# aik2mlj/polyffusion

Hardware: AMD Instinct MI355X
Metric: denoising steps/sec (8-bar prmat2c, batch 16) (higher is better)
Workload: dtype bf16x3; 1 GPU; sdf_chd8bar cond generation, batch 16 per GPU, 1000-step DDPM sampler loop body (BASELINE.json configs[1]); weights: deterministic synthetic, 41.08M params; global_batch=16, parallelism=batch-shard x1

## Files before the change

polyffusion_amd/csrc/conv_bf16x3.hip:

```cpp
#include <vector>

#include "conv_common.h"

namespace pf {

#ifdef PF_TRACE
__device__ unsigned long long g_trace[8192];
#define TR() do { if (trace_on && tslot < 2040) { g_trace[tbase + tslot++] = __builtin_amdgcn_s_memtime(); } } while (0)
#else
#define TR() do {} while (0)
#endif

typedef x3_t x3x4 __attribute__((ext_vector_type(4)));

template <int KS, int STRIDE, int TWIN, int BN>
constexpr int conv_bf3_row_pitch() {
  return (KS != 1 && STRIDE == 1 && BN >= 128) ? (TWIN * 40 + 127) / 128 * 128 : TWIN * 40;
}

#ifndef PF_KG2_RING
#define PF_KG2_RING 5
#endif
template <int KS, int BN, int KG>
constexpr bool conv_bf3_pingpong() { return KS == 3 && BN == 128 && KG == 2; }
template <int KS, int KG, int BN = 64>
constexpr int conv_bf3_wring() { return KS == 3 ? (KG == 2 && !conv_bf3_pingpong<KS, BN, KG>() ? PF_KG2_RING : 3) : 2; }

template <int KS, int STRIDE, int TH, int TW, int BN, bool SKIP, int KG = 1>
constexpr size_t conv_bf3_group_lds() {
  constexpr int THIN = (TH - 1) * STRIDE + KS, TWIN = (TW - 1) * STRIDE + KS;
  constexpr int NABUF = (KS == 1) ? 2 : 1, WRING = conv_bf3_wring<KS, KG, BN>();
  constexpr size_t main_b = (size_t)(2 * NABUF * THIN * conv_bf3_row_pitch<KS, STRIDE, TWIN, BN>() + WRING * 8 * BN * 8) * 2;
  constexpr int NB1 = BN >= 128 ? 2 : 1;
  constexpr size_t skip_b = SKIP ? (size_t)(2 * NB1 * TH * TW * 40 + NB1 * 8 * BN * 8) * 2 : 0;
  return main_b > skip_b ? main_b : skip_b;
}

template <int KS, int STRIDE, bool UPS, int TH, int TW, int BN, int PRO, int NWM, bool SKIP, int KG = 1>
__global__ __launch_bounds__(KG * NWM * 128, 2) void conv_bf3_kernel(ConvP p) {
  constexpr int NT = NWM * 128;
  constexpr int BK = 32;
  constexpr int BM = TH * TW;
  constexpr int THIN = (TH - 1) * STRIDE + KS;
  constexpr int TWIN = (TW - 1) * STRIDE + KS;
  constexpr int NPIX = THIN * TWIN;
  constexpr int PITCH = BK + 8;
  constexpr int KQ = BK / 4;
  constexpr int TOTA = NPIX * KQ;
  constexpr int NA = (TOTA + NT - 1) / NT;
  constexpr int PSTEP = NT / KQ;
  constexpr int TOTW = 8 * BN;
  constexpr int NW = TOTW / NT;
  constexpr int TAPS = KS * KS;
  constexpr int NABUF = (KS == 1) ? 2 : 1;
  constexpr int WRING = conv_bf3_wring<KS, KG, BN>();
  constexpr int WM = BM / NWM, WN = BN / 2;
  constexpr int FM = WM / 32, FN = WN / 32;
  constexpr int PAD = (KS == 3) ? 1 : 0;
  constexpr int RP = conv_bf3_row_pitch<KS, STRIDE, TWIN, BN>();
  constexpr int ABUF = THIN * RP;
  constexpr int APLANE = NABUF * ABUF;
  static_assert(TOTW % NT == 0 && FM >= 1 && FN >= 1, "bad tile");

  extern __shared__ __attribute__((aligned(16))) unsigned char smem_all[];
  const int kg = KG == 1 ? 0 : __builtin_amdgcn_readfirstlane(threadIdx.x / NT);
  unsigned char* smem_raw = smem_all + kg * conv_bf3_group_lds<KS, STRIDE, TH, TW, BN, SKIP, KG>();
  x3_t* sAh = reinterpret_cast<x3_t*>(smem_raw);
  x3_t* sAl = sAh + APLANE;
  x3_t* sW = sAl + APLANE;

  const int tid = KG == 1 ? threadIdx.x : threadIdx.x % NT, lane = tid & 63;
  const int wave = __builtin_amdgcn_readfirstlane(tid >> 6);
#ifdef PF_TRACE
  const bool trace_on = (threadIdx.x == 0) && (blockIdx.x == 0 || blockIdx.x == 301 || blockIdx.x == gridDim.x - 1);
  const int tbase = blockIdx.x == 0 ? 0 : (blockIdx.x == 301 ? 2048 : 4096);
  int tslot = 0;
  TR();
#endif
  const int wm = wave >> 1, wn = wave & 1;

  const int nwg = gridDim.x;
  int lid;
  {
    const int orig = blockIdx.x;
    const int xcd = orig & 7, q = nwg >> 3, r = nwg & 7;
    lid = (xcd < r ? xcd * (q + 1) : r * (q + 1) + (xcd - r) * q) + (orig >> 3);
  }
  int q = 0;
  if constexpr (KS == 2) { q = lid & 3; lid >>= 2; p.fold_py = q >> 1; p.fold_px = q & 1; }
  int t = fdiv(lid, p.d_ks);
  const int sidx = lid - t * p.ksplit;
  lid = t;
  int mt = fdiv(lid, p.d_nt);
  const int nti = lid - mt * p.nt;
  t = fdiv(mt, p.d_tx);
  const int tx = mt - t * p.tiles_x; mt = t;
  const int b = fdiv(mt, p.d_ty);
  const int ty = mt - b * p.tiles_y;
  const int n0 = nti * BN;
  const int oy0 = ty * TH, ox0 = tx * TW;
  conv_shared_x1(p, b);
  const int ppad = p.x1_bmod > 0 ? (b - b % p.x1_bmod) * p.Hin * p.Win : 0;
  const int iy0 = KS == 2 ? oy0 - 1 + (q >> 1) : oy0 * STRIDE - PAD, ix0 = KS == 2 ? ox0 - 1 + (q & 1) : ox0 * STRIDE - PAD;
  const int Hlog = UPS ? 2 * p.Hin : p.Hin, Wlog = UPS ? 2 * p.Win : p.Win;
  const int cin = p.c0 + p.c1;
  const int K8 = cin / 8;
  const int nsl = p.ksplit * KG, sl = sidx * KG + kg;
  const bool pow2 = (nsl & (nsl - 1)) == 0;
  const int nsh = 31 - __builtin_clz(nsl);
  const int cbeg = pow2 ? ((cin / BK) * sl) >> nsh : (cin / BK) * sl / nsl;
  const int nchunk = (pow2 ? ((cin / BK) * (sl + 1)) >> nsh : (cin / BK) * (sl + 1) / nsl) - cbeg;

  const int c4 = tid % KQ;
  int poff[NA];
  float pmu[NA], prs[NA];
#pragma unroll
  for (int i = 0; i < NA; ++i) {
    const int pix = tid / KQ + i * PSTEP;
    poff[i] = -1; pmu[i] = 0.f; prs[i] = 0.f;
    if (pix < NPIX) {
      const int hy = pix / TWIN, hx = pix % TWIN;
      const int iy = iy0 + hy, ix = ix0 + hx;
      if (iy >= 0 && iy < Hlog && ix >= 0 && ix < Wlog) {
        const int sy = UPS ? (iy >> 1) : iy, sx = UPS ? (ix >> 1) : ix;
        poff[i] = (b * p.Hin + sy) * p.Win + sx;
        if (PRO == 3) { pmu[i] = p.mean[poff[i]]; prs[i] = p.rstd[poff[i]]; }
      }
    }
  }

  f32x4 ra[NA], vsc, vsh;
  u32x4 rw[NW];
  vsc = f32x4{1.f, 1.f, 1.f, 1.f}; vsh = f32x4{0.f, 0.f, 0.f, 0.f};

  bool sc_ready = !((PRO == 1 || PRO == 2) && p.gn_s0);
  auto loadA = [&](int chunk) {
    const int cg = (cbeg + chunk) * BK;
    const float* src; int cs, co;
    if (cg < p.c0) { src = p.x0; cs = p.c0; co = cg; } else { src = p.x1; cs = p.c1; co = cg - p.c0; }
#pragma unroll
    for (int i = 0; i < NA; ++i) {
      if (KS != 1 || poff[i] >= 0) ra[i] = *reinterpret_cast<const f32x4*>(src + co + (unsigned)(max(poff[i], ppad) * cs + c4 * 4));
      else ra[i] = f32x4{0.f, 0.f, 0.f, 0.f};
    }
    if (PRO == 1 || PRO == 2) {
      const float* scp = sc_ready ? p.sc + (size_t)b * cin : p.gn_gamma;
      const float* shp = sc_ready ? p.sh + (size_t)b * cin : p.gn_beta;
      vsc = *reinterpret_cast<const f32x4*>(scp + cg + c4 * 4);
      vsh = *reinterpret_cast<const f32x4*>(shp + cg + c4 * 4);
    } else if (PRO == 3) {
      vsc = *reinterpret_cast<const f32x4*>(p.sc + cg + c4 * 4);
      vsh = *reinterpret_cast<const f32x4*>(p.sh + cg + c4 * 4);
    }
  };
  x3x4 qh[NA], ql[NA];
  auto transformPiece = [&](int i) {
    {
      f32x4 v = ra[i];
      if (poff[i] < 0) v = f32x4{0.f, 0.f, 0.f, 0.f};
      else if (PRO != 0) {
        if (PRO == 3) {
          v = (v - pmu[i]) * prs[i] * vsc + vsh;
        } else {
          v = v * vsc + vsh;
          if (PRO == 1) { v[0] = silu_f(v[0]); v[1] = silu_f(v[1]); v[2] = silu_f(v[2]); v[3] = silu_f(v[3]); }
        }
      }
      qh[i] = __builtin_convertvector(v, x3x4);
      const f32x4 hf = __builtin_convertvector(qh[i], f32x4);
      ql[i] = __builtin_convertvector(v - hf, x3x4);
    }
  };
  auto transformA = [&]() {
#pragma unroll
    for (int i = 0; i < NA; ++i) transformPiece(i);
  };
  auto writeA = [&](int buf) {
#pragma unroll
    for (int i = 0; i < NA; ++i) {
      const int pix = tid / KQ + i * PSTEP;
      if (pix < NPIX) {
        const int o = buf * ABUF + (pix / TWIN) * RP + (pix % TWIN) * PITCH + c4 * 4;
        *reinterpret_cast<x3x4*>(sAh + o) = qh[i];
        *reinterpret_cast<x3x4*>(sAl + o) = ql[i];
      }
    }
  };
  auto storeA = [&](int buf) { transformA(); writeA(buf); };
  auto loadW = [&](int chunk, int tap) {
    const size_t toff = ((size_t)tap * K8 + (size_t)(cbeg + chunk) * 4) * ((size_t)2 * p.Npad * 8);
#pragma unroll
    for (int j = 0; j < NW; ++j) {
      const int u = tid + j * NT;
      const int k8l = u / (2 * BN), plane = (u / BN) & 1, n = u % BN;
      rw[j] = *reinterpret_cast<const u32x4*>(static_cast<const x3_t*>(p.w) + ((size_t)(k8l * 2 + plane) * p.Npad + n0 + n) * 8 + toff);
    }
  };
  auto storeW = [&](int buf) {
    x3_t* dst = sW + buf * (TOTW * 8);
#pragma unroll
    for (int j = 0; j < NW; ++j) {
      *reinterpret_cast<u32x4*>(dst + (tid + j * NT) * 8) = rw[j];
    }
  };

  static_assert(NT % (2 * BN) == 0, "pieces of a thread must be whole k8 rows apart");
  const int wrow_b = 2 * p.Npad * 8 * 2;
  const __amdgpu_buffer_rsrc_t rsW = dma_resource(static_cast<const x3_t*>(p.w) + (size_t)n0 * 8);
  const int vw0 = (((tid / (2 * BN)) * 2 + ((tid / BN) & 1)) * p.Npad + tid % BN) * 16;
  auto gldsW = [&](int chunk, int tap, int buf) {
    const int toff = ((q * TAPS + tap) * K8 + (cbeg + chunk) * 4) * wrow_b;
#pragma unroll
    for (int j = 0; j < NW; ++j) {
      x3_t* l = sW + buf * (TOTW * 8) + (wave * 64 + j * NT) * 8;
      dma16(rsW, vw0, toff + j * (NT / (2 * BN)) * wrow_b, l);
    }
  };

  int hbase[FM];
#pragma unroll
  for (int fm = 0; fm < FM; ++fm) {
    const int pp = wm * WM + fm * 32 + (lane & 31);
    const int py = pp / TW, px = pp % TW;
    hbase[fm] = (py * STRIDE) * RP + (px * STRIDE) * PITCH + 8 * (lane >> 5);
  }
  const int wbase = ((lane >> 5) * 2 * BN + wn * WN + (lane & 31)) * 8;

  f32x16 acc[FM][FN];
#pragma unroll
  for (int fm = 0; fm < FM; ++fm)
#pragma unroll
    for (int fn = 0; fn < FN; ++fn)
#pragma unroll
      for (int r = 0; r < 16; ++r) acc[fm][fn][r] = 0.f;


  auto gnFused = [&]() {
    if constexpr (PRO == 1 || PRO == 2) {
      if (p.gn_s0) {
        gn_fused_prologue<KG * NT>(p, b, threadIdx.x, p.Hin * p.Win, reinterpret_cast<double*>(smem_all));
        const int cg = cbeg * BK;
        vsc = *reinterpret_cast<const f32x4*>(p.sc + (size_t)b * cin + cg + c4 * 4);
        vsh = *reinterpret_cast<const f32x4*>(p.sh + (size_t)b * cin + cg + c4 * 4);
        sc_ready = true;
      }
    }
  };
  if constexpr (KS == 1) {
    loadA(0); loadW(0, 0);
    gnFused();
    storeA(0); storeW(0);
    __syncthreads();
    for (int chunk = 0; chunk < nchunk; ++chunk) {
      const int nchunk1 = min(chunk + 1, nchunk - 1);
      loadW(nchunk1, 0);
      loadA(nchunk1);
      const int aoff = (chunk & 1) * ABUF;
      const x3_t* cW = sW + (chunk & 1) * (TOTW * 8) + wbase;
#pragma unroll
      for (int s = 0; s < BK / 16; ++s) {
        x3x8 ah[FM], al[FM], bh[FN], bl[FN];
#pragma unroll
        for (int fm = 0; fm < FM; ++fm) {
          ah[fm] = *reinterpret_cast<const x3x8*>(sAh + aoff + hbase[fm] + s * 16);
          al[fm] = *reinterpret_cast<const x3x8*>(sAl + aoff + hbase[fm] + s * 16);
        }
#pragma unroll
        for (int fn = 0; fn < FN; ++fn) {
          bh[fn] = *reinterpret_cast<const x3x8*>(cW + ((4 * s) * BN + fn * 32) * 8);
          bl[fn] = *reinterpret_cast<const x3x8*>(cW + ((4 * s + 1) * BN + fn * 32) * 8);
        }
#pragma unroll
        for (int fm = 0; fm < FM; ++fm)
#pragma unroll
          for (int fn = 0; fn < FN; ++fn) acc[fm][fn] = x3_mfma_32x32x16(al[fm], bh[fn], acc[fm][fn], 0, 0, 0);
#pragma unroll
        for (int fm = 0; fm < FM; ++fm)
#pragma unroll
          for (int fn = 0; fn < FN; ++fn) acc[fm][fn] = x3_mfma_32x32x16(ah[fm], bl[fn], acc[fm][fn], 0, 0, 0);
#pragma unroll
        for (int fm = 0; fm < FM; ++fm)
#pragma unroll
          for (int fn = 0; fn < FN; ++fn) acc[fm][fn] = x3_mfma_32x32x16(ah[fm], bh[fn], acc[fm][fn], 0, 0, 0);
      }
      storeW((chunk + 1) & 1);
      storeA((chunk + 1) & 1);
      __syncthreads();
    }
  } else {
    constexpr int NS = BK / 16;
    static_assert(NS == 2 && WRING >= 2 && WRING <= TAPS, "pipeline is written for two K steps per tap and a ring no deeper than a chunk's taps");
    constexpr bool DYN = TAPS % WRING != 0;
    constexpr int NAL = NA + (PRO != 0 ? 2 : 0);
    constexpr bool PP = conv_bf3_pingpong<KS, BN, KG>();
#pragma unroll
    for (int d = 0; d < (PP ? 2 : WRING); ++d) gldsW(0, d, d);
    TR();
    loadA(0);
    TR();
    gnFused();
    storeA(0);
    TR();
    asm volatile("s_waitcnt vmcnt(0) lgkmcnt(0)" ::: "memory");
    __builtin_amdgcn_s_barrier();
    x3x8 ah[FM], al[FM], bh[FN], bl[FN];
    unsigned abase[FM];
#pragma unroll
    for (int fm = 0; fm < FM; ++fm) abase[fm] = (unsigned)(size_t)(__attribute__((address_space(3))) x3_t*)(sAh + hbase[fm]);
    const unsigned wb = (unsigned)(size_t)(__attribute__((address_space(3))) x3_t*)(sW + wbase);
    constexpr int ALO = APLANE * 2;
    constexpr int WSLOT = TOTW * 16;
    static_assert(ALO + (2 * RP + 2 * PITCH) * 2 + 64 < 65536 && (DYN ? 1 : WRING) * WSLOT < 65536, "LDS immediates must fit 16 bits");
#define LD_AL1(I, AOFF, S) al[I] = lds_read128<ALO + ((AOFF) + (S) * 16) * 2>(abase[I])
#define LD_AH1(I, AOFF, S) ah[I] = lds_read128<((AOFF) + (S) * 16) * 2>(abase[I])
#define LD_BH1(I, SLOT, S) bh[I] = lds_read128<(DYN ? 0 : slot_##SLOT * WSLOT) + ((4 * (S)) * BN + (I) * 32) * 16>(DYN ? wb_##SLOT : wb)
#define LD_BL1(I, SLOT, S) bl[I] = lds_read128<(DYN ? 0 : slot_##SLOT * WSLOT) + ((4 * (S) + 1) * BN + (I) * 32) * 16>(DYN ? wb_##SLOT : wb)
#define LD_AL(AOFF, S) static_for<0, FM>([&](auto i) { LD_AL1(i.value, AOFF, S); })
#define LD_AH(AOFF, S) static_for<0, FM>([&](auto i) { LD_AH1(i.value, AOFF, S); })
#define LD_BH(SLOT, S) static_for<0, FN>([&](auto i) { LD_BH1(i.value, SLOT, S); })
#define LD_BL(SLOT, S) static_for<0, FN>([&](auto i) { LD_BL1(i.value, SLOT, S); })
#define SB() __builtin_amdgcn_sched_barrier(0)
#define FENCE() asm volatile("" ::: "memory")
    constexpr int G = FM * FN;
    auto GX = [&](auto&& f) {
      static_for<0, FM>([&](auto fm) { static_for<0, FN>([&](auto fn) {
        acc[fm.value][fn.value] = x3_mfma_32x32x16(al[fm.value], bh[fn.value], acc[fm.value][fn.value], 0, 0, 0);
        SB(); f(fm, fn); SB(); }); });
    };
    auto GZ = [&](auto&& f) {
      static_for<0, FN>([&](auto fn) { static_for<0, FM>([&](auto fm) {
        acc[fm.value][fn.value] = x3_mfma_32x32x16(ah[fm.value], bh[fn.value], acc[fm.value][fn.value], 0, 0, 0);
        SB(); f(fm, fn); SB(); }); });
    };
    auto GY = [&](auto&& f) {
      static_for<0, FM>([&](auto fm) { static_for<0, FN>([&](auto fn) {
        acc[fm.value][fn.value] = x3_mfma_32x32x16(ah[fm.value], bl[fn.value], acc[fm.value][fn.value], 0, 0, 0);
        SB(); f(fm, fn); SB(); }); });
    };
    auto loadApiece = [&](int chunk, int i) {
      const int cg = (cbeg + chunk) * BK;
      const float* src; int cs, co;
      if (cg < p.c0) { src = p.x0; cs = p.c0; co = cg; } else { src = p.x1; cs = p.c1; co = cg - p.c0; }
      if (i < NA) asm volatile("global_load_dwordx4 %0, %1, off" : "=v"(ra[i]) : "v"(src + co + (unsigned)(max(poff[i], ppad) * cs + c4 * 4)));
      else if (PRO == 1 || PRO == 2) {
        asm volatile("global_load_dwordx4 %0, %1, off" : "=v"(vsc) : "v"(p.sc + (size_t)b * cin + cg + c4 * 4));
        asm volatile("global_load_dwordx4 %0, %1, off" : "=v"(vsh) : "v"(p.sh + (size_t)b * cin + cg + c4 * 4));
      }
    };
    auto transformSub = [&](int i, int sub) {
      if (sub < 2) {
#pragma unroll
        for (int e = 2 * sub; e < 2 * sub + 2; ++e) {
          float v = ra[i][e];
          if (poff[i] < 0) v = 0.f;
          else if (PRO != 0) { v = v * vsc[e] + vsh[e]; if (PRO == 1) v = silu_f(v); }
          ra[i][e] = v;
        }
      } else if (sub == 2) {
        qh[i] = __builtin_convertvector(ra[i], x3x4);
      } else {
        ql[i] = __builtin_convertvector(ra[i] - __builtin_convertvector(qh[i], f32x4), x3x4);
      }
    };
    auto gldsWpiece = [&](int chunk, int tap, int buf, int j) {
      const int toff = ((q * TAPS + tap) * K8 + (cbeg + chunk) * 4) * wrow_b;
      x3_t* l = sW + buf * (TOTW * 8) + (wave * 64 + j * NT) * 8;
      dma16(rsW, vw0, toff + j * (NT / (2 * BN)) * wrow_b, l);
    };
    if constexpr (PP) {
      static_assert(WRING == 3 && TAPS == 9 && NS == 2, "ping-pong loop: ring of 3 over 9 taps");
      x3x8 ah2[NS][FM], al2[NS][FM], bh2[NS][FN], bl2[NS][FN];
      int woff[NA];
#pragma unroll
      for (int i = 0; i < NA; ++i) {
        const int pix = min(tid / KQ + i * PSTEP, NPIX - 1);
        woff[i] = (pix / TWIN) * RP + (pix % TWIN) * PITCH + c4 * 4;
      }
      if (kg) __builtin_amdgcn_s_barrier();
      for (int chunk = 0; chunk < nchunk; ++chunk) {
        const bool has_next = chunk + 1 < nchunk;
        const int chunkn = min(chunk + 1, nchunk - 1);
        static_for<0, TAPS>([&](auto tapc) {
          constexpr int tap = decltype(tapc)::value;
          constexpr int aoff = (tap / KS) * RP + (tap % KS) * PITCH;
          constexpr int slot_cur = tap % WRING, slot_ref = (tap + 2) % WRING;
          constexpr int T0 = 2, TSPAN = TAPS - 1 - T0;
          int c2 = chunk + (tap + 2) / TAPS, t2 = (tap + 2) % TAPS;
          if (c2 >= nchunk) { c2 = nchunk - 1; t2 = TAPS - 1; }
          TR();
          SB();
          static_for<0, NS>([&](auto sc_) {
            constexpr int st = decltype(sc_)::value;
            static_for<0, FM>([&](auto i) { al2[st][i.value] = lds_read128<ALO + (aoff + st * 16) * 2>(abase[i.value]); });
            static_for<0, FN>([&](auto i) { bh2[st][i.value] = lds_read128<slot_cur * WSLOT + ((4 * st) * BN + i.value * 32) * 16>(wb); });
            static_for<0, FM>([&](auto i) { ah2[st][i.value] = lds_read128<(aoff + st * 16) * 2>(abase[i.value]); });
            static_for<0, FN>([&](auto i) { bl2[st][i.value] = lds_read128<slot_cur * WSLOT + ((4 * st + 1) * BN + i.value * 32) * 16>(wb); });
          });
          static_for<0, NW>([&](auto jc) { gldsWpiece(c2, t2, slot_ref, decltype(jc)::value); });
          if constexpr (tap == 0) {
            static_for<0, NA + 1>([&](auto ic) { if (ic.value < NA || PRO != 0) loadApiece(chunkn, ic.value); });
          }
          if constexpr (tap == T0) {
            asm volatile("s_waitcnt vmcnt(%0)" ::"n"(2 * NW) : "memory");
            SB();
          }
          if (has_next) {
            static_for<0, NA>([&](auto ic) {
              constexpr int i = decltype(ic)::value;
              if constexpr (tap == T0 + (i * TSPAN) / NA) { static_for<0, 4>([&](auto sc_) { transformSub(i, decltype(sc_)::value); }); }
            });
          }
          SB();
          TR();
          asm volatile("s_waitcnt lgkmcnt(0)" ::: "memory");
          TR();
          __builtin_amdgcn_s_barrier();
          FENCE();
          SB();
          TR();
          static_for<0, NS>([&](auto sc_) {
            constexpr int st = decltype(sc_)::value;
            static_for<0, FM>([&](auto fm) { static_for<0, FN>([&](auto fn) {
              acc[fm.value][fn.value] = x3_mfma_32x32x16(al2[st][fm.value], bh2[st][fn.value], acc[fm.value][fn.value], 0, 0, 0);
              SB(); }); });
            static_for<0, FN>([&](auto fn) { static_for<0, FM>([&](auto fm) {
              acc[fm.value][fn.value] = x3_mfma_32x32x16(ah2[st][fm.value], bh2[st][fn.value], acc[fm.value][fn.value], 0, 0, 0);
              SB(); }); });
            static_for<0, FM>([&](auto fm) { static_for<0, FN>([&](auto fn) {
              acc[fm.value][fn.value] = x3_mfma_32x32x16(ah2[st][fm.value], bl2[st][fn.value], acc[fm.value][fn.value], 0, 0, 0);
              SB(); }); });
          });
          if constexpr (tap == TAPS - 1) {
            if (has_next) {
#pragma unroll
              for (int i = 0; i < NA; ++i) {
                if (tid / KQ + i * PSTEP < NPIX) {
                  *reinterpret_cast<x3x4*>(sAh + woff[i]) = qh[i];
                  *reinterpret_cast<x3x4*>(sAl + woff[i]) = ql[i];
                }
              }
            }
          }
          SB();
          TR();
          asm volatile("s_waitcnt vmcnt(%0) lgkmcnt(0)" ::"n"(NW + (tap < T0 ? NAL : 0)) : "memory");
          TR();
          __builtin_amdgcn_s_barrier();
          FENCE();
          SB();
        });
      }
      if (!kg) __builtin_amdgcn_s_barrier();
    } else {
    int rs_cur = 0;
    {
      constexpr int slot_cur = 0;
      const unsigned wb_cur = wb;
      (void)slot_cur; (void)wb_cur;
      LD_AL(0, 0); LD_BH(cur, 0); LD_AH(0, 0); LD_BL(cur, 0);
    }
    for (int chunk = 0; chunk < nchunk; ++chunk) {
      const bool has_next = chunk + 1 < nchunk;
      const int chunkn = min(chunk + 1, nchunk - 1);
      static_for<0, TAPS>([&](auto tapc) {
        constexpr int tap = decltype(tapc)::value;
        constexpr int aoff = (tap / KS) * RP + (tap % KS) * PITCH;
        constexpr int aoff1 = ((tap + 1) / KS) * RP + ((tap + 1) % KS) * PITCH;
        constexpr int slot_cur = DYN ? 0 : tap % WRING, slot_nxt = DYN ? 0 : (tap + 1) % WRING;
        const int rs_nxt = rs_cur + 1 == WRING ? 0 : rs_cur + 1;
        const int slot = DYN ? rs_cur : slot_cur;
        const unsigned wb_cur = wb + (unsigned)rs_cur * WSLOT, wb_nxt = wb + (unsigned)rs_nxt * WSLOT;
        (void)wb_cur; (void)wb_nxt; (void)slot_nxt;
        constexpr int T0 = TAPS >= 9 ? 2 : 1, TSPAN = TAPS - 1 - T0;
        int c2 = chunk + (tap + WRING) / TAPS, t2 = (tap + WRING) % TAPS;
        if (c2 >= nchunk) { c2 = nchunk - 1; t2 = TAPS - 1; }
        auto filler = [&](auto kc) {
          constexpr int k = decltype(kc)::value;
          if constexpr (tap == 0 && k < 3 * G) {
            static_for<0, NA + 1>([&](auto ic) {
              constexpr int i = decltype(ic)::value;
              if constexpr (k == (i * 3 * G) / (NA + 1)) { if (i < NA || PRO != 0) loadApiece(chunkn, i); }
            });
          }
          if constexpr (k >= 3 * G && k < 4 * G) {
            if constexpr (tap == T0 && k == 3 * G) {
              asm volatile("s_waitcnt vmcnt(%0)" ::"n"(T0 * NW) : "memory");
              SB();
            }
            if (has_next) {
              static_for<0, NA>([&](auto ic) {
                constexpr int i = decltype(ic)::value;
                if constexpr (tap == T0 + (i * TSPAN) / NA) {
                  static_for<0, 4>([&](auto sc_) {
                    constexpr int sub = decltype(sc_)::value;
                    if constexpr (k - 3 * G == (sub * G) / 4) transformSub(i, sub);
                  });
                }
              });
            }
          }
          if constexpr (k >= 4 * G && k < 5 * G) {
            static_for<0, NW>([&](auto jc) {
              constexpr int j = decltype(jc)::value;
              if constexpr (k - 4 * G == (j * G) / NW) gldsWpiece(c2, t2, slot, j);
            });
          }
        };
        TR();
        SB();
        lgkm_wait<(tap == 0) ? FM : FM + FN>(); SB();
        GX([&](auto fm, auto fn) {
          if constexpr (fn.value == FN - 1) LD_AL1(fm.value, aoff, 1);
          filler(std::integral_constant<int, 0 * G + fm.value * FN + fn.value>{});
        });
        lgkm_wait<(tap == 0) ? FM : FM + FN>(); SB();
        GZ([&](auto fm, auto fn) {
          if constexpr (fm.value == FM - 1) LD_BH1(fn.value, cur, 1);
          filler(std::integral_constant<int, 1 * G + fn.value * FM + fm.value>{});
        });
        lgkm_wait<FM + FN>(); SB();
        GY([&](auto fm, auto fn) {
          if constexpr (fn.value == FN - 1) LD_AH1(fm.value, aoff, 1);
          if constexpr (fm.value == FM - 1 && fn.value == FN - 1) LD_BL(cur, 1);
          filler(std::integral_constant<int, 2 * G + fm.value * FN + fn.value>{});
        });
        lgkm_wait<FM + FN>(); SB();
        GX([&](auto fm, auto fn) { filler(std::integral_constant<int, 3 * G + fm.value * FN + fn.value>{}); });
        SB();
        TR();
        asm volatile("s_waitcnt vmcnt(%0) lgkmcnt(0)" ::"n"((WRING - 2) * NW + (tap < WRING - 1 ? NAL : 0)) : "memory");
        TR();
        __builtin_amdgcn_s_barrier();
        FENCE();
        SB();
        TR();
        if constexpr (tap == TAPS - 1) {
          if (has_next) writeA(0);
          SB();
          GZ([&](auto fm, auto fn) {
            if constexpr (fm.value == FM - 1) LD_BH1(fn.value, nxt, 0);
            filler(std::integral_constant<int, 4 * G + fn.value * FM + fm.value>{});
          });
          GY([&](auto fm, auto fn) {
            if constexpr (fm.value == FM - 1 && fn.value == FN - 1) LD_BL(nxt, 0);
            filler(std::integral_constant<int, 5 * G + fm.value * FN + fn.value>{});
          });
          asm volatile("s_waitcnt lgkmcnt(0)" ::: "memory");
          __builtin_amdgcn_s_barrier();
          FENCE();
          LD_AL(0, 0); LD_AH(0, 0); SB();
        } else {
          GZ([&](auto fm, auto fn) {
            if constexpr (fn.value == 0) LD_AL1(fm.value, aoff1, 0);
            if constexpr (fm.value == FM - 1) LD_BH1(fn.value, nxt, 0);
            filler(std::integral_constant<int, 4 * G + fn.value * FM + fm.value>{});
          });
          GY([&](auto fm, auto fn) {
            if constexpr (fn.value == FN - 1) LD_AH1(fm.value, aoff1, 0);
            if constexpr (fm.value == FM - 1 && fn.value == FN - 1) LD_BL(nxt, 0);
            filler(std::integral_constant<int, 5 * G + fm.value * FN + fn.value>{});
          });
        }
        rs_cur = rs_nxt;
      });
    }
    }
#undef LD_AL1
#undef LD_AH1
#undef LD_BH1
#undef LD_BL1
#undef LD_AL
#undef LD_AH
#undef LD_BH
#undef LD_BL
#undef FENCE
#undef SB
    asm volatile("s_waitcnt vmcnt(0) lgkmcnt(0)" ::: "memory");
#pragma unroll
    for (int i = 0; i < NA; ++i) asm volatile("" : "+v"(ra[i]));
    asm volatile("" : "+v"(vsc), "+v"(vsh));
    if constexpr (!PP) {
    #pragma unroll
    for (int i = 0; i < FM; ++i) asm volatile("" ::"v"(al[i]), "v"(ah[i]));
    #pragma unroll
    for (int i = 0; i < FN; ++i) asm volatile("" ::"v"(bh[i]), "v"(bl[i]));
    }
    __builtin_amdgcn_sched_barrier(0);
  }

  if constexpr (SKIP) {
    if (sidx == 0) {
      constexpr int NB1 = BN >= 128 ? 2 : 1;
      constexpr int NA1 = BM * KQ / NT;
      static_assert(BM * KQ % NT == 0, "tile pixels must divide over the block");
      x3_t* a1h = reinterpret_cast<x3_t*>(smem_raw);
      x3_t* a1l = a1h + NB1 * BM * PITCH;
      x3_t* w1 = a1l + NB1 * BM * PITCH;
      int goff[NA1];
#pragma unroll
      for (int i = 0; i < NA1; ++i) {
        const int pix = tid / KQ + i * PSTEP;
        const int oy = oy0 + pix / TW, ox = ox0 + pix % TW;
        goff[i] = (oy < p.Hout && ox < p.Wout) ? (b * p.Hout + oy) * p.Wout + ox : -1;
      }
      f32x4 r1[NA1];
      u32x4 rw1[NW];
      auto load1 = [&](int chunk) {
        const int cg = chunk * BK;
        const float* src; int cs, co;
        if (cg < p.sc0) { src = p.sx0; cs = p.sc0; co = cg; } else { src = p.sx1; cs = p.sc1; co = cg - p.sc0; }
#pragma unroll
        for (int i = 0; i < NA1; ++i) {
          if (goff[i] >= 0) r1[i] = *reinterpret_cast<const f32x4*>(src + co + (unsigned)(goff[i] * cs + c4 * 4));
          else r1[i] = f32x4{0.f, 0.f, 0.f, 0.f};
        }
#pragma unroll
        for (int j = 0; j < NW; ++j) {
          const int u = tid + j * NT;
          const int k8l = u / (2 * BN), plane = (u / BN) & 1, n = u % BN;
          rw1[j] = *reinterpret_cast<const u32x4*>(static_cast<const x3_t*>(p.sw) + ((size_t)((chunk * 4 + k8l) * 2 + plane) * p.Npad + n0 + n) * 8);
        }
      };
      auto store1 = [&](int buf) {
#pragma unroll
        for (int i = 0; i < NA1; ++i) {
          const x3x4 hi = __builtin_convertvector(r1[i], x3x4);
          const x3x4 lo = __builtin_convertvector(r1[i] - __builtin_convertvector(hi, f32x4), x3x4);
          const int o = (buf * BM + tid / KQ + i * PSTEP) * PITCH + c4 * 4;
          *reinterpret_cast<x3x4*>(a1h + o) = hi;
          *reinterpret_cast<x3x4*>(a1l + o) = lo;
        }
#pragma unroll
        for (int j = 0; j < NW; ++j) *reinterpret_cast<u32x4*>(w1 + buf * (TOTW * 8) + (tid + j * NT) * 8) = rw1[j];
      };
      int arow[FM];
#pragma unroll
      for (int fm = 0; fm < FM; ++fm) arow[fm] = (wm * WM + fm * 32 + (lane & 31)) * PITCH + 8 * (lane >> 5);
      const int nchx = (p.sc0 + p.sc1) / BK;
      const int ch0 = nchx * kg / KG, nch1 = nchx * (kg + 1) / KG;
      load1(ch0);
      __syncthreads();
      store1(0);
      __syncthreads();
      for (int chunk = ch0; chunk < nch1; ++chunk) {
        if (chunk + 1 < nch1) load1(chunk + 1);
        const int cur = NB1 == 2 ? ((chunk - ch0) & 1) : 0;
        const int ao = cur * BM * PITCH;
        const x3_t* cW = w1 + cur * (TOTW * 8) + wbase;
#pragma unroll
        for (int s2 = 0; s2 < BK / 16; ++s2) {
          x3x8 ah[FM], al[FM], bh[FN], bl[FN];
#pragma unroll
          for (int fm = 0; fm < FM; ++fm) {
            ah[fm] = *reinterpret_cast<const x3x8*>(a1h + ao + arow[fm] + s2 * 16);
            al[fm] = *reinterpret_cast<const x3x8*>(a1l + ao + arow[fm] + s2 * 16);
          }
#pragma unroll
          for (int fn = 0; fn < FN; ++fn) {
            bh[fn] = *reinterpret_cast<const x3x8*>(cW + ((4 * s2) * BN + fn * 32) * 8);
            bl[fn] = *reinterpret_cast<const x3x8*>(cW + ((4 * s2 + 1) * BN + fn * 32) * 8);
          }
#pragma unroll
          for (int fm = 0; fm < FM; ++fm)
#pragma unroll
            for (int fn = 0; fn < FN; ++fn) acc[fm][fn] = x3_mfma_32x32x16(al[fm], bh[fn], acc[fm][fn], 0, 0, 0);
#pragma unroll
          for (int fm = 0; fm < FM; ++fm)
#pragma unroll
            for (int fn = 0; fn < FN; ++fn) acc[fm][fn] = x3_mfma_32x32x16(ah[fm], bl[fn], acc[fm][fn], 0, 0, 0);
#pragma unroll
          for (int fm = 0; fm < FM; ++fm)
#pragma unroll
            for (int fn = 0; fn < FN; ++fn) acc[fm][fn] = x3_mfma_32x32x16(ah[fm], bh[fn], acc[fm][fn], 0, 0, 0);
        }
        if constexpr (NB1 == 1) __syncthreads();
        if (chunk + 1 < nch1) store1(NB1 == 2 ? ((chunk + 1 - ch0) & 1) : 0);
        __syncthreads();
      }
    }
  }

  TR();
  if (p.partial) p.partial += (size_t)sidx * ((size_t)p.B * p.Hout * p.Wout) * p.N;
  if constexpr (KG == 2) {
    float* xch = reinterpret_cast<float*>(smem_all);
    __syncthreads();
    if (kg == 1) {
#pragma unroll
      for (int fm = 0; fm < FM; ++fm)
#pragma unroll
        for (int fn = 0; fn < FN; ++fn)
#pragma unroll
          for (int r = 0; r < 16; ++r) xch[((fm * FN + fn) * 16 + r) * NT + tid] = acc[fm][fn][r];
    }
    __syncthreads();
    if (kg == 0) {
#pragma unroll
      for (int fm = 0; fm < FM; ++fm)
#pragma unroll
        for (int fn = 0; fn < FN; ++fn)
#pragma unroll
          for (int r = 0; r < 16; ++r) acc[fm][fn][r] += xch[((fm * FN + fn) * 16 + r) * NT + tid];
    }
    __syncthreads();
  }
  x3_unscale(acc);
  conv_epilogue<TH, TW, BN, FM, FN, NWM>(p, acc, b, oy0, ox0, n0, wm, wn, lane, tid, reinterpret_cast<float*>(smem_all), kg == 0);
  TR();
}

__global__ __launch_bounds__(1024) void splitk_reduce_kernel(const float* __restrict__ part, int S, int M, int N, int hw,
                                                            const float* __restrict__ bias, const float* __restrict__ bias2,
                                                            const float* __restrict__ sbias, int ld_sb,
                                                            const long long* __restrict__ sb_rows, int sb_nrows,
                                                            const float* __restrict__ res, int ld_res, float* __restrict__ out,
                                                            int ld_out, float* __restrict__ stats, unsigned* amax) {
  __shared__ float red[16][64][2];
  const int tid = threadIdx.x, c = tid & 63, rg = tid >> 6;
  const int row0 = blockIdx.x * 64;
  const int b = row0 / hw, tile = (row0 % hw) / 64, ntiles = hw / 64;
  {
    const int n = blockIdx.y * 64 + c;
    float s1 = 0.f, s2 = 0.f;
    unsigned am = 0;
    if (n < N) {
      long long sr = b;
      if (sb_rows) { sr = sb_rows[b]; sr = sr < 0 ? 0 : (sr >= sb_nrows ? sb_nrows - 1 : sr); }
      const float cb = (bias ? bias[n] : 0.f) + (bias2 ? bias2[n] : 0.f) + (sbias ? sbias[(size_t)sr * ld_sb + n] : 0.f);
      for (int i = 0; i < 4; ++i) {
        const size_t m = row0 + rg + 16 * i;
        float v = cb;
        for (int s = 0; s < S; ++s) v += part[((size_t)s * M + m) * N + n];
        if (res) v += res[m * ld_res + n];
        out[m * ld_out + n] = v;
        amax_acc(am, v);
        s1 += v; s2 += v * v;
      }
    }
    amax_flush(amax, am);
    if (stats) {
      red[rg][c][0] = s1; red[rg][c][1] = s2;
      __syncthreads();
      if (rg == 0 && n < N) {
        float* dst = stats + (((size_t)b * ntiles + tile) * N + n) * 2;
        float a0 = 0.f, a1 = 0.f;
#pragma unroll
        for (int j = 0; j < 16; ++j) { a0 += red[j][c][0]; a1 += red[j][c][1]; }
        dst[0] = a0; dst[1] = a1;
      }
      __syncthreads();
    }
  }
}

template <int KS, int STRIDE, bool UPS, int TH, int TW, int BN, int PRO, int NWM = 2, bool SKIP = false, int KG = 1>
static int launch3_cfg(ConvP& p, hipStream_t stream) {
  constexpr int FMFN = (TH * TW / NWM / 32) * (BN / 2 / 32);
  constexpr size_t lds_groups = KG * conv_bf3_group_lds<KS, STRIDE, TH, TW, BN, SKIP, KG>();
  constexpr size_t lds_xch = KG == 2 ? (size_t)FMFN * 16 * NWM * 128 * 4 : 0;
  constexpr size_t lds = lds_groups > lds_xch ? lds_groups : lds_xch;
  static_assert(lds <= 160 * 1024, "LDS budget");
  p.tiles_x = cdiv(p.Wout, TW);
  p.tiles_y = cdiv(p.Hout, TH);
  p.nt = cdiv(p.Npad, BN);
  conv_fill_divs(p);
  auto kern = conv_bf3_kernel<KS, STRIDE, UPS, TH, TW, BN, PRO, NWM, SKIP, KG>;
  static std::atomic<uint64_t> attr_done{0};
  if (int rc = set_max_lds_once(reinterpret_cast<const void*>(kern), (int)lds, attr_done)) return rc;
  const int grid = p.B * p.tiles_y * p.tiles_x * p.nt * p.ksplit * (KS == 2 ? 4 : 1);
  hipLaunchKernelGGL(kern, dim3(grid), dim3(KG * NWM * 128), lds, stream, p);
  PF_CHECK_HIP(hipGetLastError());
  return PF_OK;
}

template <int KS, int STRIDE, bool UPS, int PRO>
static int dispatch_tile3(ConvP& p, int tile, hipStream_t s) {
  if constexpr (KS == 1) {
    if (tile == 0) return launch3_cfg<1, 1, false, 1, 128, 128, PRO>(p, s);
    if (tile == 1) return launch3_cfg<1, 1, false, 1, 128, 64, PRO>(p, s);
    return launch3_cfg<1, 1, false, 1, 64, 64, PRO>(p, s);
  } else if constexpr (KS == 2) {
    if (tile == 0) return launch3_cfg<2, 1, false, 8, 16, 128, PRO>(p, s);
    if (tile == 1) return launch3_cfg<2, 1, false, 8, 16, 64, PRO>(p, s);
    return launch3_cfg<2, 1, false, 4, 16, 64, PRO>(p, s);
  } else if constexpr (STRIDE == 2) {
    return launch3_cfg<3, 2, false, 4, 16, 64, PRO>(p, s);
  } else {
    if constexpr (!UPS && PRO == 1) {
      const int blocks = p.B * cdiv(p.Hout, tile == 3 ? 16 : tile == 2 ? 4 : 8) * cdiv(p.Wout, 16) * cdiv(p.Npad, tile == 0 ? 128 : 64);
      const int cus = num_cus();
      const bool kg2 = tile == 2 && p.ksplit == 1 && blocks <= cus && ((p.c0 + p.c1) / 32) % 2 == 0 && (!p.sw || ((p.sc0 + p.sc1) / 32) % 2 == 0);
      if (kg2) return p.sw ? launch3_cfg<3, 1, false, 4, 16, 64, 1, 2, true, 2>(p, s) : launch3_cfg<3, 1, false, 4, 16, 64, 1, 2, false, 2>(p, s);
      if (p.pp && tile == 0 && p.ksplit == 1 && blocks <= cus && (p.c0 + p.c1) >= 256 && ((p.c0 + p.c1) / 32) % 2 == 0 && (!p.sw || ((p.sc0 + p.sc1) / 32) % 2 == 0))
        return p.sw ? launch3_cfg<3, 1, false, 8, 16, 128, 1, 2, true, 2>(p, s) : launch3_cfg<3, 1, false, 8, 16, 128, 1, 2, false, 2>(p, s);
      if (tile == 3) return p.sw ? launch3_cfg<3, 1, false, 16, 16, 64, 1, 2, true>(p, s) : launch3_cfg<3, 1, false, 16, 16, 64, 1, 2, false>(p, s);
      if (p.sw) {
        if (tile == 0) return launch3_cfg<3, 1, false, 8, 16, 128, 1, 2, true>(p, s);
        if (tile == 1) return launch3_cfg<3, 1, false, 8, 16, 64, 1, 2, true>(p, s);
        return launch3_cfg<3, 1, false, 4, 16, 64, 1, 2, true>(p, s);
      }
    }
    if (tile == 0) return launch3_cfg<3, 1, UPS, 8, 16, 128, PRO>(p, s);
    if (tile == 1) return launch3_cfg<3, 1, UPS, 8, 16, 64, PRO>(p, s);
    return launch3_cfg<3, 1, UPS, 4, 16, 64, PRO>(p, s);
  }
}

int launch_conv_bf3(const pf_conv_args& a, hipStream_t stream) {
  if (conv_wino_eligible(a)) return launch_conv_wino(a, stream);
  ConvP p;
  memset(&p, 0, sizeof p);
  p.x0 = a.x0; p.x1 = a.x1; p.c0 = a.c0; p.c1 = a.c1;
  p.B = a.batch; p.Hin = a.hin; p.Win = a.win;
  p.Hout = a.hin; p.Wout = a.win;
  if (a.ups) { p.Hout *= 2; p.Wout *= 2; }
  if (a.stride == 2) { p.Hout = (p.Hout - 1) / 2 + 1; p.Wout = (p.Wout - 1) / 2 + 1; }
  p.w = a.w; p.N = a.n; p.Npad = (a.n + 63) / 64 * 64;
  p.sc = a.sc; p.sh = a.sh; p.mean = a.mean; p.rstd = a.rstd;
  p.bias = a.bias; p.sbias = a.sbias; p.ld_sbias = a.ld_sbias; p.res = a.res; p.ld_res = a.ld_res;
  p.sb_rows = reinterpret_cast<const long long*>(a.sbias_rows); p.sb_nrows = a.sbias_nrows;
  p.geglu = a.geglu; p.out = a.out; p.ld_out = a.ld_out; p.stats = a.stats_out;
  p.ksplit = conv_ksplit(a);
  p.pp = !a.no_pp;
  p.partial = p.ksplit > 1 ? static_cast<float*>(a.splitk_ws) : nullptr;
  p.qkv = a.qkv_planes; p.out_planes = a.out_planes;
  if (a.gn_stats0 && (a.prologue == 1 || a.prologue == 2)) {
    p.gn_s0 = a.gn_stats0; p.gn_t0 = a.gn_tiles0; p.gn_s1 = a.gn_stats1; p.gn_t1 = a.gn_tiles1;
    p.gn_gamma = a.gn_gamma; p.gn_beta = a.gn_beta; p.gn_eps = a.gn_eps; p.gn_groups = a.gn_groups;
  }
  p.sx0 = a.skip_x0; p.sc0 = a.skip_c0; p.sx1 = a.skip_x1; p.sc1 = a.skip_c1; p.sw = a.skip_w; p.bias2 = a.skip_w ? a.skip_bias : nullptr;
  p.x1_bmod = a.x1_bmod;
  p.amax = static_cast<unsigned*>(a.absmax_slot);
  const int tile = conv_pick_tile(a);
  if (a.ks == 1) {
    switch (a.prologue) {
      case 0: return dispatch_tile3<1, 1, false, 0>(p, tile, stream);
      case 2: return dispatch_tile3<1, 1, false, 2>(p, tile, stream);
      default: return dispatch_tile3<1, 1, false, 3>(p, tile, stream);
    }
  }
  if (a.ups_fold) {
    p.Hout = a.hin; p.Wout = a.win; p.fold = 1;
    return dispatch_tile3<2, 1, false, 0>(p, tile, stream);
  }
  if (a.stride == 2) return dispatch_tile3<3, 2, false, 0>(p, tile, stream);
  int rc = a.ups ? dispatch_tile3<3, 1, true, 0>(p, tile, stream) : dispatch_tile3<3, 1, false, 1>(p, tile, stream);
  if (rc != PF_OK || p.ksplit == 1) return rc;
  const int M = p.B * p.Hout * p.Wout;
  hipLaunchKernelGGL(splitk_reduce_kernel, dim3(M / 64, cdiv(p.N, 64)), dim3(1024), 0, stream, static_cast<const float*>(a.splitk_ws), p.ksplit, M, p.N,
                     p.Hout * p.Wout, p.bias, p.bias2, p.sbias, p.ld_sbias, p.sb_rows, p.sb_nrows, p.res, p.ld_res, p.out, p.ld_out, p.stats, p.amax);
  PF_CHECK_HIP(hipGetLastError());
  return PF_OK;
}

#ifdef PF_TRACE
extern "C" int pf_debug_trace_read(unsigned long long* dst, int n) {
  return hipMemcpyFromSymbol(dst, HIP_SYMBOL(g_trace), (size_t)n * 8) == hipSuccess ? 0 : -1;
}
extern "C" int pf_debug_trace_clear() {
  static unsigned long long z[8192];
  return hipMemcpyToSymbol(HIP_SYMBOL(g_trace), z, sizeof z) == hipSuccess ? 0 : -1;
}
#endif

static inline unsigned short f2bf_rne(float f) {
  unsigned int u; memcpy(&u, &f, 4);
  u += 0x7FFFu + ((u >> 16) & 1u);
  return (unsigned short)(u >> 16);
}
static inline float bf2f(unsigned short h) { unsigned int u = (unsigned int)h << 16; float f; memcpy(&f, &u, 4); return f; }

bool pack_gemm_bf3(void* dst_, const float* src, int n_src, int K, int taps, int Npad, int n_off, const int* colmap) {
  unsigned short* dst = (unsigned short*)dst_;
  bool fits = true;
  const int K8 = K / 8;
  for (int n = 0; n < n_src; ++n) {
    const int col = colmap ? colmap[n] : n_off + n;
    for (int k = 0; k < K; ++k)
      for (int t = 0; t < taps; ++t) {
        const float v = src[((size_t)n * K + k) * taps + t];
#ifdef PF_X3_F16
        const float vs = fminf(fmaxf(v * PF_X3_WS, -65504.f), 65504.f);
        fits = fits && vs == v * PF_X3_WS;
        const _Float16 fh = (_Float16)vs, fl = (_Float16)(vs - (float)fh);
        unsigned short hi, lo;
        memcpy(&hi, &fh, 2); memcpy(&lo, &fl, 2);
#else
        const unsigned short hi = f2bf_rne(v);
        const unsigned short lo = f2bf_rne(v - bf2f(hi));
#endif
        const size_t base = ((size_t)t * K8 + k / 8) * 2;
        dst[((base + 0) * Npad + col) * 8 + (k & 7)] = hi;
        dst[((base + 1) * Npad + col) * 8 + (k & 7)] = lo;
      }
  }
  return fits;
}


bool pack_upfold_bf3(void* dst, const float* src, int N, int K, int Npad) {
  std::vector<float> f((size_t)N * K * 16);
  static const int lo[2][2] = {{0, 1}, {0, 2}}, hi[2][2] = {{0, 2}, {1, 2}};
  for (size_t nk = 0; nk < (size_t)N * K; ++nk) {
    const float* w = src + nk * 9;
    for (int py = 0; py < 2; ++py)
      for (int px = 0; px < 2; ++px)
        for (int dy = 0; dy < 2; ++dy)
          for (int dx = 0; dx < 2; ++dx) {
            double acc = 0.0;
            for (int ky = lo[py][dy]; ky <= hi[py][dy]; ++ky)
              for (int kx = lo[px][dx]; kx <= hi[px][dx]; ++kx) acc += w[ky * 3 + kx];
            f[nk * 16 + (py * 2 + px) * 4 + dy * 2 + dx] = (float)acc;
          }
  }
  return pack_gemm_bf3(dst, f.data(), N, K, 16, Npad, 0, nullptr);
}

}
```

Baseline: 210.5 steps/s.

## Add 4-way in-block K-split with interleaved hi/lo LDS layout for conv

Adds a KG=4 variant of the 3x3 conv kernel that splits the reduction over channels across four wave groups inside one block, with hi and lo bf16 planes interleaved per row in LDS and a three-way LDS reduction of partial accumulators. It also enables the KG=2 split for stride-2 3x3 convs when the grid is smaller than the CU count. The aim is to raise per-CU parallelism on small-grid layers, at the cost of larger blocks, more LDS and an extra cross-group reduction. The interleaved layout changes bank access patterns, which may add LDS conflicts.

```diff
diff --git a/polyffusion_amd/csrc/conv_bf16x3.hip b/polyffusion_amd/csrc/conv_bf16x3.hip
--- a/polyffusion_amd/csrc/conv_bf16x3.hip
+++ b/polyffusion_amd/csrc/conv_bf16x3.hip
@@ -13,24 +13,35 @@
 
 typedef x3_t x3x4 __attribute__((ext_vector_type(4)));
 
-template <int KS, int STRIDE, int TWIN, int BN>
+template <int KG>
+constexpr bool conv_bf3_ilv() { return KG == 4; }
+template <int KS, int STRIDE, int TWIN, int BN, int KG = 1>
 constexpr int conv_bf3_row_pitch() {
+  if (conv_bf3_ilv<KG>()) return TWIN * 72;
   return (KS != 1 && STRIDE == 1 && BN >= 128) ? (TWIN * 40 + 127) / 128 * 128 : TWIN * 40;
 }
 
 #ifndef PF_KG2_RING
 #define PF_KG2_RING 5
 #endif
+#ifndef PF_KG4_RING
+#define PF_KG4_RING 3
+#endif
 template <int KS, int BN, int KG>
 constexpr bool conv_bf3_pingpong() { return KS == 3 && BN == 128 && KG == 2; }
-template <int KS, int KG, int BN = 64>
-constexpr int conv_bf3_wring() { return KS == 3 ? (KG == 2 && !conv_bf3_pingpong<KS, BN, KG>() ? PF_KG2_RING : 3) : 2; }
+template <int KS, int KG, int BN = 64, int STRIDE = 1>
+constexpr int conv_bf3_wring() {
+  if (KS != 3) return 2;
+  if (KG == 4) return PF_KG4_RING;
+  return KG == 2 && STRIDE == 1 && !conv_bf3_pingpong<KS, BN, KG>() ? PF_KG2_RING : 3;
+}
 
 template <int KS, int STRIDE, int TH, int TW, int BN, bool SKIP, int KG = 1>
 constexpr size_t conv_bf3_group_lds() {
   constexpr int THIN = (TH - 1) * STRIDE + KS, TWIN = (TW - 1) * STRIDE + KS;
-  constexpr int NABUF = (KS == 1) ? 2 : 1, WRING = conv_bf3_wring<KS, KG, BN>();
-  constexpr size_t main_b = (size_t)(2 * NABUF * THIN * conv_bf3_row_pitch<KS, STRIDE, TWIN, BN>() + WRING * 8 * BN * 8) * 2;
+  constexpr int NABUF = (KS == 1) ? 2 : 1, WRING = conv_bf3_wring<KS, KG, BN, STRIDE>();
+  constexpr int NPL = conv_bf3_ilv<KG>() ? 1 : 2;
+  constexpr size_t main_b = (size_t)(NPL * NABUF * THIN * conv_bf3_row_pitch<KS, STRIDE, TWIN, BN, KG>() + WRING * 8 * BN * 8) * 2;
   constexpr int NB1 = BN >= 128 ? 2 : 1;
   constexpr size_t skip_b = SKIP ? (size_t)(2 * NB1 * TH * TW * 40 + NB1 * 8 * BN * 8) * 2 : 0;
   return main_b > skip_b ? main_b : skip_b;
@@ -44,7 +55,9 @@
   constexpr int THIN = (TH - 1) * STRIDE + KS;
   constexpr int TWIN = (TW - 1) * STRIDE + KS;
   constexpr int NPIX = THIN * TWIN;
-  constexpr int PITCH = BK + 8;
+  constexpr bool ILV = conv_bf3_ilv<KG>();
+  constexpr int PITCH1 = BK + 8;
+  constexpr int PITCH = ILV ? 2 * BK + 8 : PITCH1;
   constexpr int KQ = BK / 4;
   constexpr int TOTA = NPIX * KQ;
   constexpr int NA = (TOTA + NT - 1) / NT;
@@ -53,21 +66,22 @@
   constexpr int NW = TOTW / NT;
   constexpr int TAPS = KS * KS;
   constexpr int NABUF = (KS == 1) ? 2 : 1;
-  constexpr int WRING = conv_bf3_wring<KS, KG, BN>();
+  constexpr int WRING = conv_bf3_wring<KS, KG, BN, STRIDE>();
   constexpr int WM = BM / NWM, WN = BN / 2;
   constexpr int FM = WM / 32, FN = WN / 32;
   constexpr int PAD = (KS == 3) ? 1 : 0;
-  constexpr int RP = conv_bf3_row_pitch<KS, STRIDE, TWIN, BN>();
+  constexpr int RP = conv_bf3_row_pitch<KS, STRIDE, TWIN, BN, KG>();
   constexpr int ABUF = THIN * RP;
   constexpr int APLANE = NABUF * ABUF;
-  static_assert(TOTW % NT == 0 && FM >= 1 && FN >= 1, "bad tile");
+  constexpr int LOFF = ILV ? BK : APLANE;
+  static_assert(TOTW % NT == 0 && FM >= 1 && FN >= 1 && (!ILV || KS == 3), "bad tile");
 
   extern __shared__ __attribute__((aligned(16))) unsigned char smem_all[];
   const int kg = KG == 1 ? 0 : __builtin_amdgcn_readfirstlane(threadIdx.x / NT);
   unsigned char* smem_raw = smem_all + kg * conv_bf3_group_lds<KS, STRIDE, TH, TW, BN, SKIP, KG>();
   x3_t* sAh = reinterpret_cast<x3_t*>(smem_raw);
-  x3_t* sAl = sAh + APLANE;
-  x3_t* sW = sAl + APLANE;
+  x3_t* sAl = sAh + LOFF;
+  x3_t* sW = sAh + (ILV ? 1 : 2) * APLANE;
 
   const int tid = KG == 1 ? threadIdx.x : threadIdx.x % NT, lane = tid & 63;
   const int wave = __builtin_amdgcn_readfirstlane(tid >> 6);
@@ -308,7 +322,7 @@
 #pragma unroll
     for (int fm = 0; fm < FM; ++fm) abase[fm] = (unsigned)(size_t)(__attribute__((address_space(3))) x3_t*)(sAh + hbase[fm]);
     const unsigned wb = (unsigned)(size_t)(__attribute__((address_space(3))) x3_t*)(sW + wbase);
-    constexpr int ALO = APLANE * 2;
+    constexpr int ALO = LOFF * 2;
     constexpr int WSLOT = TOTW * 16;
     static_assert(ALO + (2 * RP + 2 * PITCH) * 2 + 64 < 65536 && (DYN ? 1 : WRING) * WSLOT < 65536, "LDS immediates must fit 16 bits");
 #define LD_AL1(I, AOFF, S) al[I] = lds_read128<ALO + ((AOFF) + (S) * 16) * 2>(abase[I])
@@ -594,8 +608,8 @@
       constexpr int NA1 = BM * KQ / NT;
       static_assert(BM * KQ % NT == 0, "tile pixels must divide over the block");
       x3_t* a1h = reinterpret_cast<x3_t*>(smem_raw);
-      x3_t* a1l = a1h + NB1 * BM * PITCH;
-      x3_t* w1 = a1l + NB1 * BM * PITCH;
+      x3_t* a1l = a1h + NB1 * BM * PITCH1;
+      x3_t* w1 = a1l + NB1 * BM * PITCH1;
       int goff[NA1];
 #pragma unroll
       for (int i = 0; i < NA1; ++i) {
@@ -626,7 +640,7 @@
         for (int i = 0; i < NA1; ++i) {
           const x3x4 hi = __builtin_convertvector(r1[i], x3x4);
           const x3x4 lo = __builtin_convertvector(r1[i] - __builtin_convertvector(hi, f32x4), x3x4);
-          const int o = (buf * BM + tid / KQ + i * PSTEP) * PITCH + c4 * 4;
+          const int o = (buf * BM + tid / KQ + i * PSTEP) * PITCH1 + c4 * 4;
           *reinterpret_cast<x3x4*>(a1h + o) = hi;
           *reinterpret_cast<x3x4*>(a1l + o) = lo;
         }
@@ -635,7 +649,7 @@
       };
       int arow[FM];
 #pragma unroll
-      for (int fm = 0; fm < FM; ++fm) arow[fm] = (wm * WM + fm * 32 + (lane & 31)) * PITCH + 8 * (lane >> 5);
+      for (int fm = 0; fm < FM; ++fm) arow[fm] = (wm * WM + fm * 32 + (lane & 31)) * PITCH1 + 8 * (lane >> 5);
       const int nchx = (p.sc0 + p.sc1) / BK;
       const int ch0 = nchx * kg / KG, nch1 = nchx * (kg + 1) / KG;
       load1(ch0);
@@ -645,7 +659,7 @@
       for (int chunk = ch0; chunk < nch1; ++chunk) {
         if (chunk + 1 < nch1) load1(chunk + 1);
         const int cur = NB1 == 2 ? ((chunk - ch0) & 1) : 0;
-        const int ao = cur * BM * PITCH;
+        const int ao = cur * BM * PITCH1;
         const x3_t* cW = w1 + cur * (TOTW * 8) + wbase;
 #pragma unroll
         for (int s2 = 0; s2 < BK / 16; ++s2) {
@@ -682,25 +696,28 @@
 
   TR();
   if (p.partial) p.partial += (size_t)sidx * ((size_t)p.B * p.Hout * p.Wout) * p.N;
-  if constexpr (KG == 2) {
+  if constexpr (KG >= 2) {
+    constexpr int XG = FM * FN * 16 * NT;
     float* xch = reinterpret_cast<float*>(smem_all);
     __syncthreads();
-    if (kg == 1) {
+    if (kg) {
 #pragma unroll
       for (int fm = 0; fm < FM; ++fm)
 #pragma unroll
         for (int fn = 0; fn < FN; ++fn)
 #pragma unroll
-          for (int r = 0; r < 16; ++r) xch[((fm * FN + fn) * 16 + r) * NT + tid] = acc[fm][fn][r];
+          for (int r = 0; r < 16; ++r) xch[(kg - 1) * XG + ((fm * FN + fn) * 16 + r) * NT + tid] = acc[fm][fn][r];
     }
     __syncthreads();
     if (kg == 0) {
 #pragma unroll
-      for (int fm = 0; fm < FM; ++fm)
-#pragma unroll
-        for (int fn = 0; fn < FN; ++fn)
-#pragma unroll
-          for (int r = 0; r < 16; ++r) acc[fm][fn][r] += xch[((fm * FN + fn) * 16 + r) * NT + tid];
+      for (int g = 1; g < KG; ++g)
+#pragma unroll
+        for (int fm = 0; fm < FM; ++fm)
+#pragma unroll
+          for (int fn = 0; fn < FN; ++fn)
+#pragma unroll
+            for (int r = 0; r < 16; ++r) acc[fm][fn][r] += xch[(g - 1) * XG + ((fm * FN + fn) * 16 + r) * NT + tid];
     }
     __syncthreads();
   }
@@ -757,7 +774,7 @@
 static int launch3_cfg(ConvP& p, hipStream_t stream) {
   constexpr int FMFN = (TH * TW / NWM / 32) * (BN / 2 / 32);
   constexpr size_t lds_groups = KG * conv_bf3_group_lds<KS, STRIDE, TH, TW, BN, SKIP, KG>();
-  constexpr size_t lds_xch = KG == 2 ? (size_t)FMFN * 16 * NWM * 128 * 4 : 0;
+  constexpr size_t lds_xch = KG >= 2 ? (size_t)(KG - 1) * FMFN * 16 * NWM * 128 * 4 : 0;
   constexpr size_t lds = lds_groups > lds_xch ? lds_groups : lds_xch;
   static_assert(lds <= 160 * 1024, "LDS budget");
   p.tiles_x = cdiv(p.Wout, TW);
@@ -773,6 +790,9 @@
   return PF_OK;
 }
 
+#ifndef PF_KG_MAX
+#define PF_KG_MAX 4
+#endif
 template <int KS, int STRIDE, bool UPS, int PRO>
 static int dispatch_tile3(ConvP& p, int tile, hipStream_t s) {
   if constexpr (KS == 1) {
@@ -784,12 +804,16 @@
     if (tile == 1) return launch3_cfg<2, 1, false, 8, 16, 64, PRO>(p, s);
     return launch3_cfg<2, 1, false, 4, 16, 64, PRO>(p, s);
   } else if constexpr (STRIDE == 2) {
+    const int blocks = p.B * cdiv(p.Hout, 4) * cdiv(p.Wout, 16) * cdiv(p.Npad, 64);
+    if (PF_KG_MAX >= 2 && p.ksplit == 1 && blocks <= num_cus() && ((p.c0 + p.c1) / 32) % 2 == 0) return launch3_cfg<3, 2, false, 4, 16, 64, PRO, 2, false, 2>(p, s);
     return launch3_cfg<3, 2, false, 4, 16, 64, PRO>(p, s);
   } else {
     if constexpr (!UPS && PRO == 1) {
       const int blocks = p.B * cdiv(p.Hout, tile == 3 ? 16 : tile == 2 ? 4 : 8) * cdiv(p.Wout, 16) * cdiv(p.Npad, tile == 0 ? 128 : 64);
       const int cus = num_cus();
       const bool kg2 = tile == 2 && p.ksplit == 1 && blocks <= cus && ((p.c0 + p.c1) / 32) % 2 == 0 && (!p.sw || ((p.sc0 + p.sc1) / 32) % 2 == 0);
+      if (PF_KG_MAX >= 4 && kg2 && ((p.c0 + p.c1) / 32) % 4 == 0 && (!p.sw || ((p.sc0 + p.sc1) / 32) % 4 == 0))
+        return p.sw ? launch3_cfg<3, 1, false, 4, 16, 64, 1, 2, true, 4>(p, s) : launch3_cfg<3, 1, false, 4, 16, 64, 1, 2, false, 4>(p, s);
       if (kg2) return p.sw ? launch3_cfg<3, 1, false, 4, 16, 64, 1, 2, true, 2>(p, s) : launch3_cfg<3, 1, false, 4, 16, 64, 1, 2, false, 2>(p, s);
       if (p.pp && tile == 0 && p.ksplit == 1 && blocks <= cus && (p.c0 + p.c1) >= 256 && ((p.c0 + p.c1) / 32) % 2 == 0 && (!p.sw || ((p.sc0 + p.sc1) / 32) % 2 == 0))
         return p.sw ? launch3_cfg<3, 1, false, 8, 16, 128, 1, 2, true, 2>(p, s) : launch3_cfg<3, 1, false, 8, 16, 128, 1, 2, false, 2>(p, s);
```

After: 211.5 steps/s, median of 6. No clear change (+0.5%).
